# westlake-repl/IDvs.MoRec

Measured on AMD Instinct MI355X. Metric: user-sequences/sec end-to-end train step, SASRec+BERT-base, higher is better.
Workload: dtype fp16

## Files before the change

### idvs/morec_amd/_lib.py

```python
from __future__ import annotations

import ctypes as C
import os

import torch

_HERE = os.path.dirname(os.path.abspath(__file__))
LIB_PATH = os.environ.get("MOREC_HIP_LIB") or os.path.join(_HERE, "libmorec_hip.so")

F32, BF16, F16 = 0, 1, 2
ACT_NONE, ACT_GELU, ACT_RELU = 0, 1, 2
DACT_MUL = 3


class MorecError(RuntimeError):
    pass


class GemmDesc(C.Structure):
    _fields_ = [("M", C.c_int), ("N", C.c_int), ("K", C.c_int), ("lda", C.c_int), ("ldb", C.c_int), ("ldc", C.c_int),
                ("in_dtype", C.c_int), ("out_dtype", C.c_int), ("act", C.c_int), ("dact", C.c_int),
                ("accumulate", C.c_int), ("split_k", C.c_int), ("alpha", C.c_float), ("aux_deriv", C.c_int)]


# ... 17 lines not shown
    _fields_ = [("B", C.c_int), ("S", C.c_int), ("D", C.c_int), ("Nc", C.c_int), ("col_offset", C.c_int),
                ("dtype", C.c_int), ("dE_fp32", C.c_int), ("ws_from_fwd", C.c_int)]


class StepParams(C.Structure):
    _fields_ = [("step", C.c_int32), ("found_inf", C.c_int32), ("growth_tracker", C.c_int32), ("skipped", C.c_int32),
                ("loss_scale", C.c_float), ("inv_scale", C.c_float), ("bc1", C.c_float), ("bc2", C.c_float), ("apply", C.c_int32),
                ("pad0", C.c_int32), ("drop_seed", C.c_uint64), ("drop_seed_mixed", C.c_uint64), ("reserved", C.c_int32 * 2)]


class SwinAttnDesc(C.Structure):
    _fields_ = [("n_img", C.c_int), ("H", C.c_int), ("W", C.c_int), ("window", C.c_int), ("shift", C.c_int),
                ("heads", C.c_int), ("dh", C.c_int), ("scale", C.c_float), ("dtype", C.c_int)]


_P = C.c_void_p
_SIGS = {
    "morec_strerror": (C.c_char_p, [C.c_int]),
    "morec_version": (C.c_int, []),
    "morec_tuning_set": (C.c_int, [C.c_char_p, C.c_int]),
    "morec_det_scratch_reserve": (C.c_int, [C.c_size_t, C.c_void_p]),
    "morec_stream_wait_stream": (C.c_int, [_P, _P]),
    "morec_fold_defer_begin": (C.c_int, [_P]),
    "morec_fold_defer_active": (C.c_int, []),
    "morec_fold_flush": (C.c_int, [_P]),
    "morec_fold_defer_end": (C.c_int, []),
    "morec_fold_stats": (C.c_int, [_P]),
    "morec_gemm_nt": (C.c_int, [C.POINTER(GemmDesc), _P, _P, _P, _P, _P, _P, _P]),
    "morec_gemm_nt_colsum": (C.c_int, [C.POINTER(GemmDesc), _P, _P, _P, _P, _P, _P, _P, _P, _P]),
    "morec_gemm_colsum_workspace_bytes": (C.c_size_t, [C.c_int, C.c_int]),
    "morec_gemm_plan": (C.c_int, [C.POINTER(GemmDesc), C.c_int, C.c_int, C.c_int, C.c_int, C.c_int, C.POINTER(GemmPlanInfo)]),
    "morec_gemm_tn": (C.c_int, [_P, _P, _P, C.c_int, C.c_int, C.c_int, C.c_int, C.c_int, C.c_int, C.c_int, C.c_int, C.c_int, _P, _P]),
    "morec_gemm_tn_workspace_bytes": (C.c_size_t, [C.c_int, C.c_int, C.c_int]),
    "morec_mlp_dact_recompute_supported": (C.c_int, [C.c_int, C.c_int, C.c_int, C.c_int]),
    "morec_mlp_dact_recompute_workspace_bytes": (C.c_size_t, [C.c_int]),
    "morec_mlp_dact_recompute": (C.c_int, [_P, _P, _P, _P, _P, _P, _P, _P, C.c_int, C.c_int, C.c_int, C.c_int, _P]),
    "morec_transpose": (C.c_int, [_P, _P, C.c_int, C.c_int, C.c_int, C.c_int, C.c_int, C.c_int, _P]),
    "morec_transpose_batch": (C.c_int, [_P, C.c_int, C.c_int, C.c_int, _P]),
    "morec_cast": (C.c_int, [_P, _P, C.c_size_t, C.c_int, C.c_int, _P]),
    "morec_split_bf16x3": (C.c_int, [_P, _P, C.c_int, C.c_int, C.c_int, C.c_int, C.c_int, _P]),
    "morec_act_bwd": (C.c_int, [_P, _P, _P, C.c_size_t, C.c_int, C.c_int, _P]),
    "morec_scaled_sum": (C.c_int, [_P, _P, _P, _P, C.c_size_t, C.c_float, C.c_int, _P]),
    "morec_colsum": (C.c_int, [_P, _P, C.c_int, C.c_int, C.c_int, C.c_int, _P]),
    "morec_layernorm_fwd": (C.c_int, [_P, _P, _P, _P, C.c_int, _P, _P, C.c_float, _P, _P, _P, _P, C.c_int, C.c_int,
                                      C.c_int, C.c_float, C.c_uint64, C.c_float, C.c_uint64, _P, C.c_int, _P]),
    "morec_layernorm_bwd": (C.c_int, [_P, _P, _P, _P, _P, _P, _P, _P, _P, _P, _P, C.c_int, C.c_int, C.c_int, C.c_float,
                                      C.c_uint64, C.c_float, C.c_uint64, _P, _P, C.c_int, _P]),
    "morec_layernorm_fwd_res32": (C.c_int, [_P, _P, _P, _P, C.c_int, _P, _P, C.c_float, _P, _P, _P, _P, _P, C.c_int, C.c_int,
                                            C.c_int, C.c_float, C.c_uint64, C.c_float, C.c_uint64, _P]),
    "morec_layernorm_fwd_res32_pre": (C.c_int, [_P, _P, _P, _P, _P, _P, _P, _P, _P, C.c_float, _P, _P, _P, _P, C.c_int, C.c_int, C.c_int,
                                                C.c_float, C.c_uint64, _P]),
    "morec_layernorm_bwd_res32": (C.c_int, [_P, _P, _P, _P, _P, _P, _P, _P, _P, _P, _P, C.c_int, C.c_int, C.c_int, C.c_float,
                                            C.c_uint64, C.c_float, C.c_uint64, _P]),
    "morec_pos_grad": (C.c_int, [_P, _P, C.c_int, C.c_int, C.c_int, C.c_int, _P]),
    "morec_attn_fwd": (C.c_int, [C.POINTER(AttnDesc), _P, _P, _P, _P]),
    "morec_attn_bwd": (C.c_int, [C.POINTER(AttnDesc), _P, _P, _P, _P, _P]),
    "morec_attn_bwd_dbias": (C.c_int, [C.POINTER(AttnDesc), _P, _P, _P, _P, C.c_int, _P, _P, C.c_size_t, _P]),
    "morec_bert_embed_fwd": (C.c_int, [_P, _P, _P, _P, _P, _P, C.c_float, _P, _P, _P, _P, C.c_int, C.c_int, C.c_int,
                                       C.c_int, C.c_float, C.c_uint64, _P]),
    "morec_bert_embed_bwd": (C.c_int, [_P, _P, _P, _P, _P, C.c_int, C.c_int, C.c_int, C.c_int, C.c_int, _P, _P]),
    "morec_gather_rows": (C.c_int, [_P, _P, _P, C.c_int, C.c_int, C.c_int, _P]),
    "morec_scatter_add_rows": (C.c_int, [_P, _P, _P, C.c_int, C.c_int, C.c_int, C.c_int, _P]),
    "morec_indexed_rows_copy": (C.c_int, [_P, _P, _P, _P, C.c_int, C.c_int, C.c_int, _P]),
    "morec_strided_rows_copy": (C.c_int, [_P, _P, C.c_int, C.c_int, C.c_int, C.c_int, C.c_int, _P]),
    "morec_inbatch_ce_workspace_bytes": (C.c_size_t, [C.POINTER(CeDesc)]),
    "morec_inbatch_ce_fwd": (C.c_int, [C.POINTER(CeDesc), _P, _P, _P, _P, _P, _P, _P, _P, _P, _P, _P, _P]),
# ... 69 lines not shown
```

### idvs/morec_amd/csrc/gemm_tn.hip

```cpp
#include "gemm_core.hpp"
#include "gemm_args.hpp"

int gemm_tn8p_try_launch(const bf16* DY, const bf16* X, float* out, size_t slab_stride, int M, int N, int K, int ldy, int ldx, int ldo,
                         int mchunk, int zs, int dtype, hipStream_t s);

namespace {
constexpr int TT = 64;
constexpr int TC = 256;
constexpr int ROWB = TC * 2;
constexpr int OPB = TT * ROWB;
constexpr int STAGE = 2 * OPB;
constexpr int LDS_TN = 2 * STAGE;
constexpr int NWAVE = 16, NTHREADS = 1024;
constexpr int WN = 4, WK = 4;
constexpr int NI = 4, KI = 4;
constexpr int DPW = (TT * ROWB / 1024) / NWAVE;
typedef __attribute__((ext_vector_type(4))) short s16x4_t;
typedef __attribute__((address_space(3))) s16x4_t* lds_s16x4_ptr;

struct TnArgs {
    const bf16* DY;
    const bf16* X;
    float* C;
    int M, N, K, ldy, ldx, ldc, mchunk, tiles_n, tiles_k, atomic;
    float* slabs;
};

__device__ __forceinline__ bf16x8_t tr_frag(const char* tile, int ks, int blk) {
    const int lane = threadIdx.x & 63, c = lane & 15, g = lane >> 4;
    const int row = ks * 32 + 4 * g + (c >> 2);
    const char* p0 = tile + row * ROWB + ((blk ^ (row & 7)) * 32) + 8 * (c & 3);
    const s16x4_t lo = __builtin_amdgcn_ds_read_tr16_b64_v4i16((lds_s16x4_ptr)(p0));
    const s16x4_t hi = __builtin_amdgcn_ds_read_tr16_b64_v4i16((lds_s16x4_ptr)(p0 + 16 * ROWB));
    typedef __attribute__((ext_vector_type(8))) short s16x8_t;
    const s16x8_t v = {lo[0], lo[1], lo[2], lo[3], hi[0], hi[1], hi[2], hi[3]};
    return __builtin_bit_cast(bf16x8_t, v);
}
// ... 110 lines not shown
template <typename TO>
__global__ __launch_bounds__(256) void reduce_slabs_kernel(const float* __restrict__ slabs, TO* __restrict__ C, int N, int K,
                                                           int ldc, int nslab, int accumulate) {
    const size_t total4 = (size_t)N * K / 4;
    for (size_t i = blockIdx.x * (size_t)blockDim.x + threadIdx.x; i < total4; i += (size_t)gridDim.x * blockDim.x) {
        const size_t e = i * 4;
        const int n = (int)(e / K), k = (int)(e % K);
        float4 s = reinterpret_cast<const float4*>(slabs)[i];
        int t = 1;
        for (; t + 8 <= nslab; t += 8) {
            float4 v[8];
#pragma unroll
            for (int u = 0; u < 8; ++u) v[u] = reinterpret_cast<const float4*>(slabs + (size_t)(t + u) * N * K)[i];
#pragma unroll
            for (int u = 0; u < 8; ++u) { s.x += v[u].x; s.y += v[u].y; s.z += v[u].z; s.w += v[u].w; }
        }
        for (; t < nslab; ++t) {
            const float4 v = reinterpret_cast<const float4*>(slabs + (size_t)t * N * K)[i];
            s.x += v.x; s.y += v.y; s.z += v.z; s.w += v.w;
        }
        if constexpr (sizeof(TO) == 4) {
            float4* dst = reinterpret_cast<float4*>(C + (size_t)n * ldc + k);
            if (accumulate) {
                const float4 c = *dst;
                s.x += c.x; s.y += c.y; s.z += c.z; s.w += c.w;
            }
            *dst = s;
        } else {
            const float o[4] = {s.x, s.y, s.z, s.w};
            io<TO>::store4(C + (size_t)n * ldc + k, o);
        }
    }
}
}

extern "C" size_t morec_gemm_tn_workspace_bytes(int N, int K, int split_m) {
    return split_m > 1 ? (size_t)split_m * N * K * sizeof(float) : 0;
}

int gemm_tn_launch(const void* DY, const void* X, void* C, int c_dtype, int M, int N, int K, int ldy, int ldx, int ldc, int dtype, int split_m,
                   int accumulate, float* workspace, void* stream) {
    if (!DY || !X || !C || M <= 0 || N <= 0 || K <= 0) return MOREC_E_ARG;
    if (!is_h16(dtype)) return MOREC_E_UNSUPPORTED;
    if (c_dtype != MOREC_F32 && c_dtype != dtype) return MOREC_E_DTYPE;
    if (N % 8 || K % 8 || ldy % 8 || ldx % 8 || ldc % 4 || !aligned16(DY) || !aligned16(X) || !aligned16(C)) return MOREC_E_ALIGN;
    if (split_m > 1 && !accumulate && !workspace) return MOREC_E_ARG;
    TnArgs a;
    a.DY = reinterpret_cast<const bf16*>(DY); a.X = reinterpret_cast<const bf16*>(X); a.C = reinterpret_cast<float*>(C);
    a.M = M; a.N = N; a.K = K; a.ldy = ldy; a.ldx = ldx; a.ldc = ldc; a.atomic = accumulate ? 1 : 0;
    const int split = split_m < 1 ? 1 : split_m;
    int mchunk = (M + split - 1) / split;
    mchunk = ((mchunk + TT - 1) / TT) * TT;
    a.mchunk = mchunk;
    const int zs = (M + mchunk - 1) / mchunk;
    a.tiles_n = (N + TC - 1) / TC; a.tiles_k = (K + TC - 1) / TC;
    a.slabs = (zs > 1 && workspace) ? workspace : nullptr;
    if (a.slabs && (K % 4 || !aligned16(workspace))) return MOREC_E_ALIGN;
    if (c_dtype != MOREC_F32 && (!a.slabs || accumulate)) return MOREC_E_UNSUPPORTED;
    if (zs > 1 && !a.slabs && !accumulate) return MOREC_E_ARG;
    int r8 = MOREC_E_UNSUPPORTED;
    if (a.slabs)
        r8 = gemm_tn8p_try_launch(a.DY, a.X, a.slabs, (size_t)N * K, M, N, K, ldy, ldx, K, mchunk, zs, dtype, reinterpret_cast<hipStream_t>(stream));
    else if (zs == 1 && !accumulate)
        r8 = gemm_tn8p_try_launch(a.DY, a.X, a.C, 0, M, N, K, ldy, ldx, ldc, mchunk, 1, dtype, reinterpret_cast<hipStream_t>(stream));
    if (r8 != MOREC_E_UNSUPPORTED && r8 != MOREC_OK) return r8;
    if (r8 == MOREC_E_UNSUPPORTED) {
        by_h16(dtype, [&](auto* t) {
            using T = MOREC_TAG_T(t);
            static const hipError_t attr_rc = hipFuncSetAttribute(reinterpret_cast<const void*>(&gemm_tn_kernel<T>), hipFuncAttributeMaxDynamicSharedMemorySize, LDS_TN);
            (void)attr_rc;
            hipLaunchKernelGGL(gemm_tn_kernel<T>, dim3(a.tiles_n * a.tiles_k, 1, zs), dim3(NTHREADS), LDS_TN, reinterpret_cast<hipStream_t>(stream), a);
        });
        MOREC_CHECK_LAUNCH();
    }
    if (a.slabs) {
        const size_t total4 = (size_t)N * K / 4;
        const unsigned blocks = (unsigned)((total4 + 255) / 256 > 2048 ? 2048 : (total4 + 255) / 256);
        if (c_dtype == MOREC_F32)
            hipLaunchKernelGGL(reduce_slabs_kernel<float>, dim3(blocks), dim3(256), 0, reinterpret_cast<hipStream_t>(stream), a.slabs, a.C, N,
                               K, ldc, zs, accumulate ? 1 : 0);
        else if (c_dtype == MOREC_BF16)
            hipLaunchKernelGGL(reduce_slabs_kernel<bf16>, dim3(blocks), dim3(256), 0, reinterpret_cast<hipStream_t>(stream), a.slabs,
                               reinterpret_cast<bf16*>(C), N, K, ldc, zs, 0);
        else
            hipLaunchKernelGGL(reduce_slabs_kernel<f16>, dim3(blocks), dim3(256), 0, reinterpret_cast<hipStream_t>(stream), a.slabs,
                               reinterpret_cast<f16*>(C), N, K, ldc, zs, 0);
        MOREC_CHECK_LAUNCH();
// ... 9 lines not shown
```

### idvs/morec_amd/csrc/gemm_tn8p.hip

```cpp
#include "gemm_core.hpp"
#include "gemm_args.hpp"


namespace {
typedef __attribute__((ext_vector_type(16))) float f32x16_t;
typedef __attribute__((ext_vector_type(4))) unsigned int u32x4_t;
typedef __attribute__((ext_vector_type(4))) short s16x4_t;
typedef __attribute__((ext_vector_type(8))) short s16x8_t;
typedef __attribute__((address_space(3))) s16x4_t* lds_s16x4_ptr;

constexpr int TT = 64;
constexpr int ROWB = 256;
constexpr int HALF_BYTES = TT * ROWB;
constexpr int OP_BYTES = 2 * HALF_BYTES;
constexpr int BUF_BYTES = 2 * OP_BYTES;
constexpr int LDS_MAIN = 2 * BUF_BYTES;
constexpr int SLICE = 4096;
constexpr int LDS_TOTAL = LDS_MAIN + 8 * SLICE;
constexpr int THREADS = 512;

struct TnArgs8 {
    const bf16* DY;
    const bf16* X;
    float* out;
// ... 9 lines not shown
__device__ __forceinline__ void bar() {
    pin();
    __builtin_amdgcn_s_barrier();
    pin();
}
template <int REM, int W1, int W0>
__device__ __forceinline__ void vm_wait_tail() {
    vm_wait<(REM >= 2 ? 8 : (REM == 1 ? W1 : W0))>();
}

struct Ctx {
    __amdgpu_buffer_rsrc_t ry, rx;
    uint32_t y1[2], y2[2], x1[2], x2[2];
    int tok[2];
    int dpiece;
    int ay[2], ax;
    uint32_t vmask;
};

__device__ __forceinline__ void dma2(__amdgpu_buffer_rsrc_t rs, const uint32_t (&o)[2], const int (&tok)[2], int left, int soff, char* dst) {
    const uint32_t o0 = tok[0] < left ? o[0] : 0x80000000u;
    const uint32_t o1 = tok[1] < left ? o[1] : 0x80000000u;
    __builtin_amdgcn_raw_ptr_buffer_load_lds(rs, (lptr_t)dst, 16, o0, soff, 0, 0);
    __builtin_amdgcn_raw_ptr_buffer_load_lds(rs, (lptr_t)(dst + 1024), 16, o1, soff, 0, 0);
}

__device__ __forceinline__ bf16x8_t tr_frag(const char* smem, int addr, int ks) {
    const s16x4_t lo = __builtin_amdgcn_ds_read_tr16_b64_v4i16((lds_s16x4_ptr)(smem + addr + (16 * ks) * ROWB));
    const s16x4_t hi = __builtin_amdgcn_ds_read_tr16_b64_v4i16((lds_s16x4_ptr)(smem + addr + (16 * ks + 4) * ROWB));
    const s16x8_t v = {lo[0], lo[1], lo[2], lo[3], hi[0], hi[1], hi[2], hi[3]};
    return __builtin_bit_cast(bf16x8_t, v);
}

template <typename T16, int N0, int KQ, bool SKIP>
__device__ __forceinline__ void mfma_quadrant(f32x16_t (&acc)[4][2], const bf16x8_t (&fy)[2][4], const bf16x8_t (&fx)[4], uint32_t vm) {
    if constexpr (SKIP) {
        if (!(vm & (16u << KQ))) return;
        const bool a = (vm >> N0) & 1u, b = (vm >> (N0 + 1)) & 1u;
        if (!(a && b)) {
            if (!(a || b)) return;
            __builtin_amdgcn_s_setprio(1);
            if (a) {
#pragma unroll
                for (int ks = 0; ks < 4; ++ks) acc[N0][KQ] = h16<T16>::mma32(fx[ks], fy[0][ks], acc[N0][KQ]);
            } else {
#pragma unroll
                for (int ks = 0; ks < 4; ++ks) acc[N0 + 1][KQ] = h16<T16>::mma32(fx[ks], fy[1][ks], acc[N0 + 1][KQ]);
            }
            __builtin_amdgcn_s_setprio(0);
            return;
        }
    }
    __builtin_amdgcn_s_setprio(1);
#pragma unroll
    for (int ks = 0; ks < 4; ++ks)
#pragma unroll
        for (int ni = 0; ni < 2; ++ni)
            acc[N0 + ni][KQ] = h16<T16>::mma32(fx[ks], fy[ni][ks], acc[N0 + ni][KQ]);
    __builtin_amdgcn_s_setprio(0);
}

template <typename T16, int REM, bool SKIP>
__device__ __forceinline__ void stage(char* smem, const Ctx& c, int cb, int soy, int sox, int dy_step, int dx_step, int left,
                                      f32x16_t (&acc)[4][2]) {
    char* cur = smem + cb;
    char* oth = smem + (cb ^ BUF_BYTES);
    bf16x8_t fy[2][4], fx0[4], fx1[4];
    const int ay0 = cb + c.ay[0], ay1 = cb + c.ay[1], ax = cb + OP_BYTES + c.ax;
#pragma unroll
    for (int ks = 0; ks < 4; ++ks) fx0[ks] = tr_frag(smem, ax, ks);
#pragma unroll
    for (int ks = 0; ks < 4; ++ks) {
        fy[0][ks] = tr_frag(smem, ay0, ks);
        fy[1][ks] = tr_frag(smem, ay1, ks);
    }
    if constexpr (REM >= 1) dma2(c.rx, c.x2, c.tok, left - TT, sox + dx_step, oth + OP_BYTES + HALF_BYTES + c.dpiece);
    pin();
    vm_wait_tail<REM, 8, 2>();
    bar();
    mfma_quadrant<T16, 0, 0, SKIP>(acc, fy, fx0, c.vmask);
    bar();
#pragma unroll
    for (int ks = 0; ks < 4; ++ks) fx1[ks] = tr_frag(smem, ax + HALF_BYTES, ks);
    if constexpr (REM >= 1) dma2(c.ry, c.y2, c.tok, left - TT, soy + dy_step, oth + HALF_BYTES + c.dpiece);
    pin();
    vm_wait_tail<REM, 8, 0>();
    bar();
    mfma_quadrant<T16, 0, 1, SKIP>(acc, fy, fx1, c.vmask);
    bar();
#pragma unroll
    for (int ks = 0; ks < 4; ++ks) {
        fy[0][ks] = tr_frag(smem, ay0 + HALF_BYTES, ks);
        fy[1][ks] = tr_frag(smem, ay1 + HALF_BYTES, ks);
    }
    if constexpr (REM >= 2) dma2(c.ry, c.y1, c.tok, left - 2 * TT, soy + 2 * dy_step, cur + c.dpiece);
    pin();
    vm_wait_tail<REM, 6, 0>();
    bar();
    mfma_quadrant<T16, 2, 1, SKIP>(acc, fy, fx1, c.vmask);
    bar();
    if constexpr (REM >= 2) dma2(c.rx, c.x1, c.tok, left - 2 * TT, sox + 2 * dx_step, cur + OP_BYTES + c.dpiece);
    pin();
    vm_wait_tail<REM, 4, 0>();
    bar();
    mfma_quadrant<T16, 2, 0, SKIP>(acc, fy, fx0, c.vmask);
    bar();
}

template <typename T16, bool SKIP>
__device__ __forceinline__ void tn_body(const TnArgs8& p, char* smem, const bf16* __restrict__ DYt, const bf16* __restrict__ Xt, int n0, int k0,
                                        int mbeg, int mend, float* __restrict__ dst) {
    const int lane = threadIdx.x & 63;
    const int wave = __builtin_amdgcn_readfirstlane(threadIdx.x >> 6);
    const int wr = wave >> 2, wc = wave & 3;
    const int nt = (mend - mbeg + TT - 1) / TT;
    Ctx c;
    {
#pragma unroll
        for (int j = 0; j < 2; ++j) {
            const int t = 8 * wave + 4 * j + (lane >> 4);
            const int lc = (lane & 15) ^ (4 * (t & 3));
            const int ycol = (lc < 8 ? lc * 8 : 128 + (lc - 8) * 8);
            const int xcol = (lc >> 2) * 64 + (lc & 3) * 8;
            c.tok[j] = t;
            c.y1[j] = (uint32_t)(t * p.ldy + min(n0 + ycol, p.N - 8) - n0) * 2u;
            c.y2[j] = (uint32_t)(t * p.ldy + min(n0 + ycol + 64, p.N - 8) - n0) * 2u;
            c.x1[j] = (uint32_t)(t * p.ldx + min(k0 + xcol, p.K - 8) - k0) * 2u;
            c.x2[j] = (uint32_t)(t * p.ldx + min(k0 + xcol + 32, p.K - 8) - k0) * 2u;
        }
        const long ybytes = (long)(p.M - mbeg) * p.ldy * 2, xbytes = (long)(p.M - mbeg) * p.ldx * 2;
        c.ry = __builtin_amdgcn_make_buffer_rsrc((void*)DYt, 0, (int)min(ybytes, 0x7fffffffL), 0x00020000);
        c.rx = __builtin_amdgcn_make_buffer_rsrc((void*)Xt, 0, (int)min(xbytes, 0x7fffffffL), 0x00020000);
        c.dpiece = 8 * wave * ROWB;
        const int rr = (lane & 15) >> 2, cgrp = (lane >> 4) & 1, h = lane >> 5;
        const int rowoff = (8 * h + rr) * ROWB + 8 * (lane & 3);
#pragma unroll
        for (int cg = 0; cg < 2; ++cg) c.ay[cg] = rowoff + (((wr * 4 + cg * 2 + cgrp) ^ (2 * rr)) << 5);
        c.ax = rowoff + (((wc * 2 + cgrp) ^ (2 * rr)) << 5);
        uint32_t vm = 0;
#pragma unroll
        for (int i = 0; i < 4; ++i) vm |= (n0 + wr * 128 + i * 32 < p.N) ? (1u << i) : 0u;
#pragma unroll
        for (int j = 0; j < 2; ++j) vm |= (k0 + wc * 64 + j * 32 < p.K) ? (16u << j) : 0u;
        c.vmask = __builtin_amdgcn_readfirstlane(vm);
    }
    const int dy_step = TT * p.ldy * 2, dx_step = TT * p.ldx * 2;
    const int left0 = mend - mbeg;
    dma2(c.ry, c.y1, c.tok, left0, 0, smem + c.dpiece);
    dma2(c.rx, c.x1, c.tok, left0, 0, smem + OP_BYTES + c.dpiece);
    dma2(c.rx, c.x2, c.tok, left0, 0, smem + OP_BYTES + HALF_BYTES + c.dpiece);
    dma2(c.ry, c.y2, c.tok, left0, 0, smem + HALF_BYTES + c.dpiece);
    dma2(c.ry, c.y1, c.tok, left0 - TT, dy_step, smem + BUF_BYTES + c.dpiece);
    dma2(c.rx, c.x1, c.tok, left0 - TT, dx_step, smem + BUF_BYTES + OP_BYTES + c.dpiece);
    pin();

    f32x16_t acc[4][2];
#pragma unroll
    for (int i = 0; i < 4; ++i)
#pragma unroll
        for (int j = 0; j < 2; ++j)
#pragma unroll
            for (int v = 0; v < 16; ++v) acc[i][j][v] = 0.f;
    vm_wait<8>();
    bar();
    if (wr == 1) bar();
    int cb = 0, t = 0;
    for (; t < nt - 2; ++t) {
        stage<T16, 2, SKIP>(smem, c, cb, t * dy_step, t * dx_step, dy_step, dx_step, left0 - t * TT, acc);
        cb ^= BUF_BYTES;
    }
    stage<T16, 1, SKIP>(smem, c, cb, t * dy_step, t * dx_step, dy_step, dx_step, left0 - t * TT, acc);
    stage<T16, 0, SKIP>(smem, c, cb ^ BUF_BYTES, (t + 1) * dy_step, (t + 1) * dx_step, dy_step, dx_step, left0 - (t + 1) * TT, acc);
    if (wr == 0) bar();

    const int r5 = lane & 31, hh = lane >> 5;
    char* ws = smem + LDS_MAIN + wave * SLICE;
    const int rs_row = lane >> 3, rs_slot = lane & 7;
    const int rs_off = rs_row * 128 + ((rs_slot ^ (rs_row & 7)) << 4);
    const int nrows = min(256, p.N - n0);
    const long obytes = (long)nrows * p.ldo * 4;
    const __amdgpu_buffer_rsrc_t ro = __builtin_amdgcn_make_buffer_rsrc((void*)(dst + (size_t)n0 * p.ldo), 0, (int)min(obytes, 0x7fffffffL), 0x00020000);
    auto wfence = [&]() {
        __builtin_amdgcn_fence(__ATOMIC_RELEASE, "wavefront");
        __builtin_amdgcn_wave_barrier();
        __builtin_amdgcn_fence(__ATOMIC_ACQUIRE, "wavefront");
    };
#pragma unroll
    for (int Ni = 0; Ni < 4; ++Ni) {
#pragma unroll
        for (int Ki = 0; Ki < 2; ++Ki) {
            pin();
#pragma unroll
            for (int g = 0; g < 4; ++g) {
                const int slot = 2 * g + hh;
                *reinterpret_cast<float4*>(ws + r5 * 128 + ((slot ^ (r5 & 7)) << 4)) =
                    make_float4(acc[Ni][Ki][4 * g], acc[Ni][Ki][4 * g + 1], acc[Ni][Ki][4 * g + 2], acc[Ni][Ki][4 * g + 3]);
            }
            wfence();
            u32x4_t q[4];
#pragma unroll
            for (int i = 0; i < 4; ++i) q[i] = *reinterpret_cast<const u32x4_t*>(ws + rs_off + i * 1024);
            const int kcol = k0 + wc * 64 + Ki * 32 + rs_slot * 4;
            const uint32_t lo = kcol < p.K ? (uint32_t)((rs_row * p.ldo + kcol) * 4) : 0x80000000u;
#pragma unroll
            for (int i = 0; i < 4; ++i)
                __builtin_amdgcn_raw_buffer_store_b128(q[i], ro, lo + (uint32_t)((wr * 128 + Ni * 32 + 8 * i) * p.ldo * 4), 0, 0);
            wfence();
        }
    }
}

template <typename T16, bool SKIP>
__global__ __launch_bounds__(THREADS) void gemm_tn8p_kernel(TnArgs8 p) {
    extern __shared__ __attribute__((aligned(16))) char smem[];
    const int tiles = p.tiles_n * p.tiles_k;
    const int item = xcd_remap(blockIdx.x, tiles * p.zs);
    const int z = item / tiles, wg = item - z * tiles;
    const int n0 = (wg / p.tiles_k) * 256, k0 = (wg % p.tiles_k) * 256;
    const int mbeg = z * p.mchunk, mend = min(p.M, mbeg + p.mchunk);
    tn_body<T16, SKIP>(p, smem, p.DY + (size_t)mbeg * p.ldy + n0, p.X + (size_t)mbeg * p.ldx + k0, n0, k0, mbeg, mend,
            p.out + (size_t)z * p.slab_stride);
}
}

int gemm_tn8p_try_launch(const bf16* DY, const bf16* X, float* out, size_t slab_stride, int M, int N, int K, int ldy, int ldx, int ldo,
                         int mchunk, int zs, int dtype, hipStream_t s) {
    const int mode = tuning().gemm8p;
    if (mode == 1) return MOREC_E_UNSUPPORTED;
    if (N % 8 || K % 8 || ldo % 4) return MOREC_E_UNSUPPORTED;
    if (mchunk % TT || mchunk < 2 * TT) return MOREC_E_UNSUPPORTED;
    if (M - (zs - 1) * (long)mchunk < 2 * TT && zs > 1) return MOREC_E_UNSUPPORTED;
    if (zs == 1 && M < 2 * TT) return MOREC_E_UNSUPPORTED;
    const int tiles_n = (N + 255) / 256, tiles_k = (K + 255) / 256;
    if (mode != 2) {
        if (mchunk < 8 * TT) return MOREC_E_UNSUPPORTED;
    }
    if ((long)M * ldy * 2 >= 0x7fffffffL || (long)M * ldx * 2 >= 0x7fffffffL) return MOREC_E_UNSUPPORTED;
    TnArgs8 a;
    a.DY = DY; a.X = X; a.out = out; a.M = M; a.N = N; a.K = K; a.ldy = ldy; a.ldx = ldx; a.ldo = ldo; a.mchunk = mchunk;
    a.tiles_n = tiles_n; a.tiles_k = tiles_k; a.zs = zs; a.slab_stride = slab_stride;
    if (!by_h16(dtype, [&](auto* t) {
            using T = MOREC_TAG_T(t);
            static const hipError_t attr_rc = hipFuncSetAttribute(reinterpret_cast<const void*>(&gemm_tn8p_kernel<T, false>), hipFuncAttributeMaxDynamicSharedMemorySize, LDS_TOTAL);
            static const hipError_t attr_rc2 = hipFuncSetAttribute(reinterpret_cast<const void*>(&gemm_tn8p_kernel<T, true>), hipFuncAttributeMaxDynamicSharedMemorySize, LDS_TOTAL);
            (void)attr_rc; (void)attr_rc2;
            if (tuning().tn8p_skip && ((N % 256 != 0 && N % 256 <= 224) || (K % 256 != 0 && K % 256 <= 224)))
                hipLaunchKernelGGL((gemm_tn8p_kernel<T, true>), dim3(tiles_n * tiles_k * zs), dim3(THREADS), LDS_TOTAL, s, a);
            else
                hipLaunchKernelGGL((gemm_tn8p_kernel<T, false>), dim3(tiles_n * tiles_k * zs), dim3(THREADS), LDS_TOTAL, s, a);
        }))
        return MOREC_E_UNSUPPORTED;
    MOREC_CHECK_LAUNCH();
    return MOREC_OK;
}
```

### idvs/morec_amd/csrc/tuning.hip

```cpp
#include <stdlib.h>
#include <string.h>
#include "common.hpp"

namespace {
enum Handling {
    RAW,
    FLAG,
    TMR,
    RESERVE,
    TAIL_BIAS,
    MFMA,
    AT_LEAST_1,
    NOT_CHAR_0,
    IS_CHAR_1,
    EPI,
};
struct Row {
    const char* key;
    const char* env;
    int Tuning::*field;
    int def;
    Handling how;
};
const Row ROWS[] = {
    {"gemm8p", "MOREC_GEMM8P", &Tuning::gemm8p, 0, RAW},
    {"gemm2w", "MOREC_GEMM2W", &Tuning::gemm2w, 0, RAW},
    {"gemm_small", "MOREC_GEMM_SMALL", &Tuning::gemm_small, 0, RAW},
    {"gemm_skinny", "MOREC_GEMM_SKINNY", &Tuning::gemm_skinny, 0, RAW},
    {"ce8p", "MOREC_CE8P", &Tuning::ce8p, 0, RAW},
    {"gemm8p_tmr", "MOREC_GEMM8P_TMR", &Tuning::gemm8p_tmr, 1, TMR},
    {"gemm8p_ngroup", "MOREC_GEMM8P_NGROUP", &Tuning::gemm8p_ngroup, -1, RAW},
    {"gemm8p_reserve_cus", "MOREC_GEMM8P_RESERVE_CUS", &Tuning::gemm8p_reserve_cus, 0, RESERVE},
    {"gemm8p_tail_split", "MOREC_GEMM8P_TAIL_SPLIT", &Tuning::gemm8p_tail_split, 0, FLAG},
    {"gemm8p_tail_bias", nullptr, &Tuning::gemm8p_tail_bias, 2, TAIL_BIAS},
    {"gemm8p_mfma", "MOREC_GEMM8P_MFMA", &Tuning::gemm8p_mfma, 0, MFMA},
    {"gemm8p_debug", "MOREC_GEMM8P_DEBUG", &Tuning::gemm8p_debug, 0, RAW},
    {"gemm8p_stamps_lo", nullptr, &Tuning::gemm8p_stamps_lo, 0, RAW},
    {"gemm8p_stamps_hi", nullptr, &Tuning::gemm8p_stamps_hi, 0, RAW},
    {"deterministic", "MOREC_DETERMINISTIC", &Tuning::deterministic, 0, FLAG},
    {"fold_defer", "MOREC_FOLD_DEFER", &Tuning::fold_defer, 1, FLAG},
    {nullptr, "MOREC_GEMM_TILE", &Tuning::gemm_tile, 0, RAW},
    {nullptr, "MOREC_GEMM_EPI", &Tuning::gemm_epi, 2, EPI},
    {nullptr, "MOREC_GEMM2W_STAGGER", &Tuning::gemm2w_stagger, 0, RAW},
    {nullptr, "MOREC_TN8P_SKIP", &Tuning::tn8p_skip, 1, FLAG},
    {nullptr, "MOREC_ATTN_MFMA64", &Tuning::attn_mfma64, 1, NOT_CHAR_0},
    {nullptr, "MOREC_ATTN_F32_MFMA", &Tuning::attn_f32_mfma, 1, NOT_CHAR_0},
    {nullptr, "MOREC_SWIN_WPW_MIN", &Tuning::swin_wpw_min, 8, AT_LEAST_1},
    {nullptr, "MOREC_SWIN_BWD_WIDE", &Tuning::swin_bwd_wide, 1, RAW},
    {nullptr, "MOREC_QUIET", &Tuning::quiet, 0, IS_CHAR_1},
};

int handled(Handling how, int v) {
    switch (how) {
        case FLAG: return v != 0;
        case TMR: return (v == 0 || v == 1 || v == 224 || v == 192) ? v : 1;
        case RESERVE: return v < 0 ? 0 : v > 128 ? 128 : v;
        case TAIL_BIAS: return v < 0 ? 0 : v > 16 ? 16 : v;
        case MFMA: return (v == 16 || v == 32) ? v : 0;
        case AT_LEAST_1: return v < 1 ? 1 : v;
        default: return v;
    }
}

Tuning& table() {
    static Tuning t = [] {
        Tuning x{};
        for (const Row& r : ROWS) {
            const char* e = r.env ? getenv(r.env) : nullptr;
// ... 44 lines not shown
```

### idvs/morec_amd/csrc/tuning.hpp

```cpp
#pragma once

struct Tuning {
    int gemm8p, gemm2w, gemm_small, gemm_skinny, ce8p;
    int gemm8p_tmr;
    int gemm8p_ngroup;
    int gemm8p_reserve_cus;
    int gemm8p_tail_split, gemm8p_tail_bias;
    int gemm8p_mfma;
    int gemm8p_debug;
    int gemm8p_stamps_lo, gemm8p_stamps_hi;
    int deterministic;
    int fold_defer;
    int gemm_tile;
    int gemm_epi;
    int gemm2w_stagger;
    int tn8p_skip;
    int attn_mfma64;
    int attn_f32_mfma;
    int swin_wpw_min;
    int swin_bwd_wide;
    int quiet;

    unsigned long long gemm8p_stamps() const {
        return ((unsigned long long)(unsigned)gemm8p_stamps_hi << 32) | (unsigned)gemm8p_stamps_lo;
    }
};

const Tuning& tuning();

int device_cu_count();
int gemm8p_cu_count();
```

### include/morec_hip.h

```cpp
#ifndef MOREC_HIP_H
#define MOREC_HIP_H

#include <stddef.h>
#include <stdint.h>

#ifdef __cplusplus
extern "C" {
#endif

#define MOREC_F32 0
#define MOREC_BF16 1
#define MOREC_F16 2

#define MOREC_OK 0
#define MOREC_E_ARG (-1)
#define MOREC_E_ALIGN (-2)
#define MOREC_E_UNSUPPORTED (-3)
#define MOREC_E_DTYPE (-4)
#define MOREC_E_COMM (-5)

#define MOREC_ACT_NONE 0
#define MOREC_ACT_GELU 1
#define MOREC_ACT_RELU 2
#define MOREC_DACT_MUL 3
// ... 24 lines not shown
int morec_gemm_nt(const morec_gemm_desc* d, const void* A, const void* B, void* C, const float* bias,
                  void* aux_out, const void* dact_in, void* stream);

size_t morec_gemm_colsum_workspace_bytes(int M, int N);
int morec_gemm_nt_colsum(const morec_gemm_desc* d, const void* A, const void* B, void* C, const float* bias,
                         void* aux_out, const void* dact_in, float* colsum_out, float* workspace, void* stream);

#define MOREC_GEMM_UNSUPPORTED 0
#define MOREC_GEMM_SKINNY 1
#define MOREC_GEMM_SKINNY_WIDE 2
#define MOREC_GEMM_TWO_W 3
#define MOREC_GEMM_EIGHT_P 4
#define MOREC_GEMM_SMALL 5
#define MOREC_GEMM_GENERIC 6
typedef struct {
    int family;
    int mode;
    int tile_rows, tile_cols;
    int ngroup;
    int colsum_fused;
    const char* family_name;
} morec_gemm_plan_info;
int morec_gemm_plan(const morec_gemm_desc* d, int has_bias, int has_aux, int has_dact_in, int has_colsum, int n_cu,
                    morec_gemm_plan_info* out);

int morec_mlp_dact_recompute_supported(int M, int N, int K, int dtype);
size_t morec_mlp_dact_recompute_workspace_bytes(int N);
int morec_mlp_dact_recompute(const void* dY, const void* W2t, const void* X, const void* W1, const float* b1, void* dU,
                             float* colsum_out, float* workspace, int M, int N, int K, int dtype, void* stream);

int morec_gemm_tn(const void* DY, const void* X, float* C, int M, int N, int K, int ldy, int ldx, int ldc, int dtype,
                  int split_m, int accumulate, float* workspace, void* stream);
size_t morec_gemm_tn_workspace_bytes(int N, int K, int split_m);

int morec_transpose(const void* in, void* out, int R, int C, int ld_in, int ld_out, int in_dtype, int out_dtype,
                    void* stream);

typedef struct {
    const void* src;
    void* dst;
    int rows, cols;
    int ld_src, ld_dst;
    int tile0;
    int reserved;
} morec_transpose_item;
int morec_transpose_batch(const morec_transpose_item* items, int n_items, int n_tiles, int dtype, void* stream);
int morec_cast(const void* in, void* out, size_t n, int in_dtype, int out_dtype, void* stream);
int morec_split_bf16x3(const float* in, void* out, int R, int C, int ld_in, int ld_out, int lo_slot, void* stream);
int morec_act_bwd(const void* dy, const void* pre, void* out, size_t n, int act, int dtype, void* stream);
int morec_scaled_sum(const void* x0, const void* x1, const void* x2, void* out, size_t n, float scale, int dtype, void* stream);
int morec_colsum(const void* in, float* out, int M, int N, int ld, int dtype, void* stream);

int morec_layernorm_fwd(const void* x, const float* bias, const void* res, const float* pos, int pos_period,
                        const float* gamma, const float* beta, float eps, void* z_out, void* y, float* mean,
                        float* rstd, int M, int N, int dtype, float p_in, uint64_t seed_in, float p_out,
                        uint64_t seed_out, const float* rowscale, int rows_per_scale, void* stream);
int morec_layernorm_bwd(const void* dy_a, const void* dy_b, const void* z, const float* mean, const float* rstd,
                        const float* gamma, void* dz, void* dzd, float* dgamma, float* dbeta, float* dbias, int M, int N,
                        int dtype, float p_in, uint64_t seed_in, float p_out, uint64_t seed_out, const void* dres,
                        const float* rowscale, int rows_per_scale, void* stream);

int morec_layernorm_fwd_res32(const void* x16, const float* bias, const float* res32, const float* pos, int pos_period, const float* gamma,
                              const float* beta, float eps, float* z32, float* y32, void* y16, float* mean, float* rstd, int M, int N,
                              int dtype16, float p_in, uint64_t seed_in, float p_out, uint64_t seed_out, void* stream);
int morec_layernorm_fwd_res32_pre(const void* x16, const float* bias, const float* res_z32, const float* res_mean, const float* res_rstd,
                                  const float* res_gamma, const float* res_beta, const float* gamma, const float* beta, float eps, float* z32,
// ... 147 lines not shown
```

Baseline: 3720.

## Add 16x16 MFMA variant for TN weight-gradient GEMM kernel

Adds a 16x16x32 MFMA path to the 8-phase TN (weight-gradient) GEMM kernel. It brings new LDS transpose-read fragment addressing, a different swizzle, a split accumulator layout and its own epilogue store. An auto heuristic picks 16x16 for fp16, and for bf16 when the tile count is small. The skip-masked variant stays on 32x32. A plan query API and a tuning override are also exposed. The aim is better MFMA throughput or latency hiding for these shapes, at the cost of more LDS reads per MFMA and more kernel variants.

```diff
diff --git a/idvs/morec_amd/_lib.py b/idvs/morec_amd/_lib.py
--- a/idvs/morec_amd/_lib.py
+++ b/idvs/morec_amd/_lib.py
@@ -73,6 +73,7 @@
     "morec_gemm_plan": (C.c_int, [C.POINTER(GemmDesc), C.c_int, C.c_int, C.c_int, C.c_int, C.c_int, C.POINTER(GemmPlanInfo)]),
     "morec_gemm_tn": (C.c_int, [_P, _P, _P, C.c_int, C.c_int, C.c_int, C.c_int, C.c_int, C.c_int, C.c_int, C.c_int, C.c_int, _P, _P]),
     "morec_gemm_tn_workspace_bytes": (C.c_size_t, [C.c_int, C.c_int, C.c_int]),
+    "morec_gemm_tn_plan": (C.c_int, [C.c_int, C.c_int, C.c_int, C.c_int, C.c_int, C.POINTER(C.c_int), C.POINTER(C.c_int)]),
     "morec_mlp_dact_recompute_supported": (C.c_int, [C.c_int, C.c_int, C.c_int, C.c_int]),
     "morec_mlp_dact_recompute_workspace_bytes": (C.c_size_t, [C.c_int]),
     "morec_mlp_dact_recompute": (C.c_int, [_P, _P, _P, _P, _P, _P, _P, _P, C.c_int, C.c_int, C.c_int, C.c_int, _P]),
diff --git a/idvs/morec_amd/csrc/gemm_tn.hip b/idvs/morec_amd/csrc/gemm_tn.hip
--- a/idvs/morec_amd/csrc/gemm_tn.hip
+++ b/idvs/morec_amd/csrc/gemm_tn.hip
@@ -3,6 +3,7 @@
 
 int gemm_tn8p_try_launch(const bf16* DY, const bf16* X, float* out, size_t slab_stride, int M, int N, int K, int ldy, int ldx, int ldo,
                          int mchunk, int zs, int dtype, hipStream_t s);
+int gemm_tn8p_plan(int M, int N, int K, int ldy, int ldx, int ldo, int mchunk, int zs, int dtype, int* skip, int* mfma);
 
 namespace {
 constexpr int TT = 64;
@@ -179,6 +180,28 @@
         }
     }
 }
+inline void tn_chunks(int M, int split_m, int* mchunk, int* zs) {
+    const int split = split_m < 1 ? 1 : split_m;
+    int mc = (M + split - 1) / split;
+    mc = ((mc + TT - 1) / TT) * TT;
+    *mchunk = mc;
+    *zs = (M + mc - 1) / mc;
+}
+}
+
+extern "C" int morec_gemm_tn_plan(int M, int N, int K, int split_m, int dtype, int* family, int* mfma) {
+    if (M <= 0 || N <= 0 || K <= 0 || !family || !mfma) return MOREC_E_ARG;
+    *family = 0;
+    *mfma = 16;
+    if (!is_h16(dtype)) return MOREC_E_UNSUPPORTED;
+    if (N % 8 || K % 8) return MOREC_E_ALIGN;
+    int mchunk, zs, skip = 0, mf = 16;
+    tn_chunks(M, split_m, &mchunk, &zs);
+    if (gemm_tn8p_plan(M, N, K, N, K, K, mchunk, zs, dtype, &skip, &mf) == MOREC_OK) {
+        *family = skip ? 2 : 1;
+        *mfma = mf;
+    }
+    return MOREC_OK;
 }
 
 extern "C" size_t morec_gemm_tn_workspace_bytes(int N, int K, int split_m) {
@@ -195,11 +218,9 @@
     TnArgs a;
     a.DY = reinterpret_cast<const bf16*>(DY); a.X = reinterpret_cast<const bf16*>(X); a.C = reinterpret_cast<float*>(C);
     a.M = M; a.N = N; a.K = K; a.ldy = ldy; a.ldx = ldx; a.ldc = ldc; a.atomic = accumulate ? 1 : 0;
-    const int split = split_m < 1 ? 1 : split_m;
-    int mchunk = (M + split - 1) / split;
-    mchunk = ((mchunk + TT - 1) / TT) * TT;
+    int mchunk, zs;
+    tn_chunks(M, split_m, &mchunk, &zs);
     a.mchunk = mchunk;
-    const int zs = (M + mchunk - 1) / mchunk;
     a.tiles_n = (N + TC - 1) / TC; a.tiles_k = (K + TC - 1) / TC;
     a.slabs = (zs > 1 && workspace) ? workspace : nullptr;
     if (a.slabs && (K % 4 || !aligned16(workspace))) return MOREC_E_ALIGN;
diff --git a/idvs/morec_amd/csrc/gemm_tn8p.hip b/idvs/morec_amd/csrc/gemm_tn8p.hip
--- a/idvs/morec_amd/csrc/gemm_tn8p.hip
+++ b/idvs/morec_amd/csrc/gemm_tn8p.hip
@@ -65,15 +65,47 @@
     return __builtin_bit_cast(bf16x8_t, v);
 }
 
-template <typename T16, int N0, int KQ, bool SKIP>
-__device__ __forceinline__ void mfma_quadrant(f32x16_t (&acc)[4][2], const bf16x8_t (&fy)[2][4], const bf16x8_t (&fx)[4], uint32_t vm) {
+__device__ __forceinline__ bf16x8_t tr_frag16(const char* smem, int addr, int ks) {
+    const s16x4_t lo = __builtin_amdgcn_ds_read_tr16_b64_v4i16((lds_s16x4_ptr)(smem + addr + (32 * ks) * ROWB));
+    const s16x4_t hi = __builtin_amdgcn_ds_read_tr16_b64_v4i16((lds_s16x4_ptr)(smem + addr + (32 * ks + 16) * ROWB));
+    const s16x8_t v = {lo[0], lo[1], lo[2], lo[3], hi[0], hi[1], hi[2], hi[3]};
+    return __builtin_bit_cast(bf16x8_t, v);
+}
+template <int MF>
+__device__ __forceinline__ bf16x8_t frag(const char* smem, int addr, int i) {
+    if constexpr (MF == 32) return tr_frag(smem, addr, i);
+    else return tr_frag16(smem, addr ^ ((i & 1) << 5), i >> 1);
+}
+
+struct Acc16 {
+    f32x4_t q[4];
+};
+template <int MF>
+using acc_t = std::conditional_t<MF == 16, Acc16, f32x16_t>;
+
+template <typename T16, int NI0, int NIN, int KQ>
+__device__ __forceinline__ void mfma16_run(Acc16 (&acc)[4][2], const bf16x8_t (&fy)[2][4], const bf16x8_t (&fx)[4]) {
+#pragma unroll
+    for (int ks = 0; ks < 2; ++ks)
+#pragma unroll
+        for (int ni = NI0; ni < NI0 + NIN; ++ni)
+#pragma unroll
+            for (int sb = 0; sb < 4; ++sb)
+                acc[ni][KQ].q[sb] = h16<T16>::mma16(fx[2 * ks + (sb & 1)], fy[ni & 1][2 * ks + (sb >> 1)], acc[ni][KQ].q[sb]);
+}
+
+template <typename T16, int N0, int KQ, bool SKIP, int MF>
+__device__ __forceinline__ void mfma_quadrant(acc_t<MF> (&acc)[4][2], const bf16x8_t (&fy)[2][4], const bf16x8_t (&fx)[4], uint32_t vm) {
     if constexpr (SKIP) {
         if (!(vm & (16u << KQ))) return;
         const bool a = (vm >> N0) & 1u, b = (vm >> (N0 + 1)) & 1u;
         if (!(a && b)) {
             if (!(a || b)) return;
             __builtin_amdgcn_s_setprio(1);
-            if (a) {
+            if constexpr (MF == 16) {
+                if (a) mfma16_run<T16, N0, 1, KQ>(acc, fy, fx);
+                else mfma16_run<T16, N0 + 1, 1, KQ>(acc, fy, fx);
+            } else if (a) {
 #pragma unroll
                 for (int ks = 0; ks < 4; ++ks) acc[N0][KQ] = h16<T16>::mma32(fx[ks], fy[0][ks], acc[N0][KQ]);
             } else {
@@ -85,6 +117,8 @@
         }
     }
     __builtin_amdgcn_s_setprio(1);
+    if constexpr (MF == 16) mfma16_run<T16, N0, 2, KQ>(acc, fy, fx);
+    else
 #pragma unroll
     for (int ks = 0; ks < 4; ++ks)
 #pragma unroll
@@ -93,54 +127,54 @@
     __builtin_amdgcn_s_setprio(0);
 }
 
-template <typename T16, int REM, bool SKIP>
+template <typename T16, int REM, bool SKIP, int MF>
 __device__ __forceinline__ void stage(char* smem, const Ctx& c, int cb, int soy, int sox, int dy_step, int dx_step, int left,
-                                      f32x16_t (&acc)[4][2]) {
+                                      acc_t<MF> (&acc)[4][2]) {
     char* cur = smem + cb;
     char* oth = smem + (cb ^ BUF_BYTES);
     bf16x8_t fy[2][4], fx0[4], fx1[4];
     const int ay0 = cb + c.ay[0], ay1 = cb + c.ay[1], ax = cb + OP_BYTES + c.ax;
 #pragma unroll
-    for (int ks = 0; ks < 4; ++ks) fx0[ks] = tr_frag(smem, ax, ks);
+    for (int ks = 0; ks < 4; ++ks) fx0[ks] = frag<MF>(smem, ax, ks);
 #pragma unroll
     for (int ks = 0; ks < 4; ++ks) {
-        fy[0][ks] = tr_frag(smem, ay0, ks);
-        fy[1][ks] = tr_frag(smem, ay1, ks);
+        fy[0][ks] = frag<MF>(smem, ay0, ks);
+        fy[1][ks] = frag<MF>(smem, ay1, ks);
     }
     if constexpr (REM >= 1) dma2(c.rx, c.x2, c.tok, left - TT, sox + dx_step, oth + OP_BYTES + HALF_BYTES + c.dpiece);
     pin();
     vm_wait_tail<REM, 8, 2>();
     bar();
-    mfma_quadrant<T16, 0, 0, SKIP>(acc, fy, fx0, c.vmask);
-    bar();
-#pragma unroll
-    for (int ks = 0; ks < 4; ++ks) fx1[ks] = tr_frag(smem, ax + HALF_BYTES, ks);
+    mfma_quadrant<T16, 0, 0, SKIP, MF>(acc, fy, fx0, c.vmask);
+    bar();
+#pragma unroll
+    for (int ks = 0; ks < 4; ++ks) fx1[ks] = frag<MF>(smem, ax + HALF_BYTES, ks);
     if constexpr (REM >= 1) dma2(c.ry, c.y2, c.tok, left - TT, soy + dy_step, oth + HALF_BYTES + c.dpiece);
     pin();
     vm_wait_tail<REM, 8, 0>();
     bar();
-    mfma_quadrant<T16, 0, 1, SKIP>(acc, fy, fx1, c.vmask);
+    mfma_quadrant<T16, 0, 1, SKIP, MF>(acc, fy, fx1, c.vmask);
     bar();
 #pragma unroll
     for (int ks = 0; ks < 4; ++ks) {
-        fy[0][ks] = tr_frag(smem, ay0 + HALF_BYTES, ks);
-        fy[1][ks] = tr_frag(smem, ay1 + HALF_BYTES, ks);
+        fy[0][ks] = frag<MF>(smem, ay0 + HALF_BYTES, ks);
+        fy[1][ks] = frag<MF>(smem, ay1 + HALF_BYTES, ks);
     }
     if constexpr (REM >= 2) dma2(c.ry, c.y1, c.tok, left - 2 * TT, soy + 2 * dy_step, cur + c.dpiece);
     pin();
     vm_wait_tail<REM, 6, 0>();
     bar();
-    mfma_quadrant<T16, 2, 1, SKIP>(acc, fy, fx1, c.vmask);
+    mfma_quadrant<T16, 2, 1, SKIP, MF>(acc, fy, fx1, c.vmask);
     bar();
     if constexpr (REM >= 2) dma2(c.rx, c.x1, c.tok, left - 2 * TT, sox + 2 * dx_step, cur + OP_BYTES + c.dpiece);
     pin();
     vm_wait_tail<REM, 4, 0>();
     bar();
-    mfma_quadrant<T16, 2, 0, SKIP>(acc, fy, fx0, c.vmask);
-    bar();
-}
-
-template <typename T16, bool SKIP>
+    mfma_quadrant<T16, 2, 0, SKIP, MF>(acc, fy, fx0, c.vmask);
+    bar();
+}
+
+template <typename T16, bool SKIP, int MF>
 __device__ __forceinline__ void tn_body(const TnArgs8& p, char* smem, const bf16* __restrict__ DYt, const bf16* __restrict__ Xt, int n0, int k0,
                                         int mbeg, int mend, float* __restrict__ dst) {
     const int lane = threadIdx.x & 63;
@@ -152,7 +186,7 @@
 #pragma unroll
         for (int j = 0; j < 2; ++j) {
             const int t = 8 * wave + 4 * j + (lane >> 4);
-            const int lc = (lane & 15) ^ (4 * (t & 3));
+            const int lc = (lane & 15) ^ (MF == 16 ? 2 * (t & 7) : 4 * (t & 3));
             const int ycol = (lc < 8 ? lc * 8 : 128 + (lc - 8) * 8);
             const int xcol = (lc >> 2) * 64 + (lc & 3) * 8;
             c.tok[j] = t;
@@ -165,11 +199,19 @@
         c.ry = __builtin_amdgcn_make_buffer_rsrc((void*)DYt, 0, (int)min(ybytes, 0x7fffffffL), 0x00020000);
         c.rx = __builtin_amdgcn_make_buffer_rsrc((void*)Xt, 0, (int)min(xbytes, 0x7fffffffL), 0x00020000);
         c.dpiece = 8 * wave * ROWB;
+        if constexpr (MF == 16) {
+            const int row = 4 * (lane >> 4) + ((lane & 15) >> 2);
+            const int rowoff = row * ROWB + 8 * (lane & 3);
+#pragma unroll
+            for (int cg = 0; cg < 2; ++cg) c.ay[cg] = rowoff + (((wr * 4 + cg * 2) ^ (row & 7)) << 5);
+            c.ax = rowoff + (((wc * 2) ^ (row & 7)) << 5);
+        } else {
         const int rr = (lane & 15) >> 2, cgrp = (lane >> 4) & 1, h = lane >> 5;
         const int rowoff = (8 * h + rr) * ROWB + 8 * (lane & 3);
 #pragma unroll
         for (int cg = 0; cg < 2; ++cg) c.ay[cg] = rowoff + (((wr * 4 + cg * 2 + cgrp) ^ (2 * rr)) << 5);
         c.ax = rowoff + (((wc * 2 + cgrp) ^ (2 * rr)) << 5);
+        }
         uint32_t vm = 0;
 #pragma unroll
         for (int i = 0; i < 4; ++i) vm |= (n0 + wr * 128 + i * 32 < p.N) ? (1u << i) : 0u;
@@ -187,23 +229,26 @@
     dma2(c.rx, c.x1, c.tok, left0 - TT, dx_step, smem + BUF_BYTES + OP_BYTES + c.dpiece);
     pin();
 
-    f32x16_t acc[4][2];
+    acc_t<MF> acc[4][2];
 #pragma unroll
     for (int i = 0; i < 4; ++i)
 #pragma unroll
         for (int j = 0; j < 2; ++j)
 #pragma unroll
-            for (int v = 0; v < 16; ++v) acc[i][j][v] = 0.f;
+            for (int v = 0; v < 16; ++v) {
+                if constexpr (MF == 16) acc[i][j].q[v >> 2][v & 3] = 0.f;
+                else acc[i][j][v] = 0.f;
+            }
     vm_wait<8>();
     bar();
     if (wr == 1) bar();
     int cb = 0, t = 0;
     for (; t < nt - 2; ++t) {
-        stage<T16, 2, SKIP>(smem, c, cb, t * dy_step, t * dx_step, dy_step, dx_step, left0 - t * TT, acc);
+        stage<T16, 2, SKIP, MF>(smem, c, cb, t * dy_step, t * dx_step, dy_step, dx_step, left0 - t * TT, acc);
         cb ^= BUF_BYTES;
     }
-    stage<T16, 1, SKIP>(smem, c, cb, t * dy_step, t * dx_step, dy_step, dx_step, left0 - t * TT, acc);
-    stage<T16, 0, SKIP>(smem, c, cb ^ BUF_BYTES, (t + 1) * dy_step, (t + 1) * dx_step, dy_step, dx_step, left0 - (t + 1) * TT, acc);
+    stage<T16, 1, SKIP, MF>(smem, c, cb, t * dy_step, t * dx_step, dy_step, dx_step, left0 - t * TT, acc);
+    stage<T16, 0, SKIP, MF>(smem, c, cb ^ BUF_BYTES, (t + 1) * dy_step, (t + 1) * dx_step, dy_step, dx_step, left0 - (t + 1) * TT, acc);
     if (wr == 0) bar();
 
     const int r5 = lane & 31, hh = lane >> 5;
@@ -223,12 +268,21 @@
 #pragma unroll
         for (int Ki = 0; Ki < 2; ++Ki) {
             pin();
+            if constexpr (MF == 16) {
+#pragma unroll
+                for (int sb = 0; sb < 4; ++sb) {
+                    const int row = 16 * (sb >> 1) + (lane & 15), slot = 4 * (sb & 1) + (lane >> 4);
+                    *reinterpret_cast<float4*>(ws + row * 128 + ((slot ^ (row & 7)) << 4)) =
+                        make_float4(acc[Ni][Ki].q[sb][0], acc[Ni][Ki].q[sb][1], acc[Ni][Ki].q[sb][2], acc[Ni][Ki].q[sb][3]);
+                }
+            } else {
 #pragma unroll
             for (int g = 0; g < 4; ++g) {
                 const int slot = 2 * g + hh;
                 *reinterpret_cast<float4*>(ws + r5 * 128 + ((slot ^ (r5 & 7)) << 4)) =
                     make_float4(acc[Ni][Ki][4 * g], acc[Ni][Ki][4 * g + 1], acc[Ni][Ki][4 * g + 2], acc[Ni][Ki][4 * g + 3]);
             }
+            }
             wfence();
             u32x4_t q[4];
 #pragma unroll
@@ -243,7 +297,7 @@
     }
 }
 
-template <typename T16, bool SKIP>
+template <typename T16, bool SKIP, int MF>
 __global__ __launch_bounds__(THREADS) void gemm_tn8p_kernel(TnArgs8 p) {
     extern __shared__ __attribute__((aligned(16))) char smem[];
     const int tiles = p.tiles_n * p.tiles_k;
@@ -251,36 +305,65 @@
     const int z = item / tiles, wg = item - z * tiles;
     const int n0 = (wg / p.tiles_k) * 256, k0 = (wg % p.tiles_k) * 256;
     const int mbeg = z * p.mchunk, mend = min(p.M, mbeg + p.mchunk);
-    tn_body<T16, SKIP>(p, smem, p.DY + (size_t)mbeg * p.ldy + n0, p.X + (size_t)mbeg * p.ldx + k0, n0, k0, mbeg, mend,
+    tn_body<T16, SKIP, MF>(p, smem, p.DY + (size_t)mbeg * p.ldy + n0, p.X + (size_t)mbeg * p.ldx + k0, n0, k0, mbeg, mend,
             p.out + (size_t)z * p.slab_stride);
 }
 }
 
-int gemm_tn8p_try_launch(const bf16* DY, const bf16* X, float* out, size_t slab_stride, int M, int N, int K, int ldy, int ldx, int ldo,
-                         int mchunk, int zs, int dtype, hipStream_t s) {
-    const int mode = tuning().gemm8p;
+static int tn8p_mfma_auto(int N, int K, int dtype, int skip) {
+    if (skip) return 32;
+    if (dtype == MOREC_F16) return 16;
+    return ((N + 255) / 256) * ((K + 255) / 256) <= 9 ? 16 : 32;
+}
+
+int gemm_tn8p_plan(int M, int N, int K, int ldy, int ldx, int ldo, int mchunk, int zs, int dtype, int* skip, int* mfma) {
+    const Tuning& t = tuning();
+    const int mode = t.gemm8p;
     if (mode == 1) return MOREC_E_UNSUPPORTED;
+    if (!is_h16(dtype)) return MOREC_E_UNSUPPORTED;
     if (N % 8 || K % 8 || ldo % 4) return MOREC_E_UNSUPPORTED;
     if (mchunk % TT || mchunk < 2 * TT) return MOREC_E_UNSUPPORTED;
     if (M - (zs - 1) * (long)mchunk < 2 * TT && zs > 1) return MOREC_E_UNSUPPORTED;
     if (zs == 1 && M < 2 * TT) return MOREC_E_UNSUPPORTED;
-    const int tiles_n = (N + 255) / 256, tiles_k = (K + 255) / 256;
     if (mode != 2) {
         if (mchunk < 8 * TT) return MOREC_E_UNSUPPORTED;
     }
     if ((long)M * ldy * 2 >= 0x7fffffffL || (long)M * ldx * 2 >= 0x7fffffffL) return MOREC_E_UNSUPPORTED;
+    *skip = t.tn8p_skip && ((N % 256 != 0 && N % 256 <= 224) || (K % 256 != 0 && K % 256 <= 224));
+    *mfma = t.gemm_tn8p_mfma ? t.gemm_tn8p_mfma : tn8p_mfma_auto(N, K, dtype, *skip);
+    return MOREC_OK;
+}
+
+int gemm_tn8p_try_launch(const bf16* DY, const bf16* X, float* out, size_t slab_stride, int M, int N, int K, int ldy, int ldx, int ldo,
+                         int mchunk, int zs, int dtype, hipStream_t s) {
+    int skip = 0, mfma = 32;
+    if (gemm_tn8p_plan(M, N, K, ldy, ldx, ldo, mchunk, zs, dtype, &skip, &mfma) != MOREC_OK) return MOREC_E_UNSUPPORTED;
+    const int tiles_n = (N + 255) / 256, tiles_k = (K + 255) / 256;
     TnArgs8 a;
     a.DY = DY; a.X = X; a.out = out; a.M = M; a.N = N; a.K = K; a.ldy = ldy; a.ldx = ldx; a.ldo = ldo; a.mchunk = mchunk;
     a.tiles_n = tiles_n; a.tiles_k = tiles_k; a.zs = zs; a.slab_stride = slab_stride;
+    auto launch = [&](auto kernel) {
+        hipLaunchKernelGGL(kernel, dim3(tiles_n * tiles_k * zs), dim3(THREADS), LDS_TOTAL, s, a);
+    };
     if (!by_h16(dtype, [&](auto* t) {
             using T = MOREC_TAG_T(t);
-            static const hipError_t attr_rc = hipFuncSetAttribute(reinterpret_cast<const void*>(&gemm_tn8p_kernel<T, false>), hipFuncAttributeMaxDynamicSharedMemorySize, LDS_TOTAL);
-            static const hipError_t attr_rc2 = hipFuncSetAttribute(reinterpret_cast<const void*>(&gemm_tn8p_kernel<T, true>), hipFuncAttributeMaxDynamicSharedMemorySize, LDS_TOTAL);
-            (void)attr_rc; (void)attr_rc2;
-            if (tuning().tn8p_skip && ((N % 256 != 0 && N % 256 <= 224) || (K % 256 != 0 && K % 256 <= 224)))
-                hipLaunchKernelGGL((gemm_tn8p_kernel<T, true>), dim3(tiles_n * tiles_k * zs), dim3(THREADS), LDS_TOTAL, s, a);
-            else
-                hipLaunchKernelGGL((gemm_tn8p_kernel<T, false>), dim3(tiles_n * tiles_k * zs), dim3(THREADS), LDS_TOTAL, s, a);
+            static const hipError_t attr_rc = [] {
+                hipError_t rc = hipSuccess;
+                for (const void* k : {reinterpret_cast<const void*>(&gemm_tn8p_kernel<T, false, 32>), reinterpret_cast<const void*>(&gemm_tn8p_kernel<T, true, 32>),
+                                      reinterpret_cast<const void*>(&gemm_tn8p_kernel<T, false, 16>), reinterpret_cast<const void*>(&gemm_tn8p_kernel<T, true, 16>)}) {
+                    const hipError_t r = hipFuncSetAttribute(k, hipFuncAttributeMaxDynamicSharedMemorySize, LDS_TOTAL);
+                    if (r != hipSuccess) rc = r;
+                }
+                return rc;
+            }();
+            (void)attr_rc;
+            if (mfma == 16) {
+                if (skip) launch(gemm_tn8p_kernel<T, true, 16>);
+                else launch(gemm_tn8p_kernel<T, false, 16>);
+            } else {
+                if (skip) launch(gemm_tn8p_kernel<T, true, 32>);
+                else launch(gemm_tn8p_kernel<T, false, 32>);
+            }
         }))
         return MOREC_E_UNSUPPORTED;
     MOREC_CHECK_LAUNCH();
diff --git a/idvs/morec_amd/csrc/tuning.hip b/idvs/morec_amd/csrc/tuning.hip
--- a/idvs/morec_amd/csrc/tuning.hip
+++ b/idvs/morec_amd/csrc/tuning.hip
@@ -34,6 +34,7 @@
     {"gemm8p_tail_split", "MOREC_GEMM8P_TAIL_SPLIT", &Tuning::gemm8p_tail_split, 0, FLAG},
     {"gemm8p_tail_bias", nullptr, &Tuning::gemm8p_tail_bias, 2, TAIL_BIAS},
     {"gemm8p_mfma", "MOREC_GEMM8P_MFMA", &Tuning::gemm8p_mfma, 0, MFMA},
+    {"gemm_tn8p_mfma", "MOREC_GEMM_TN8P_MFMA", &Tuning::gemm_tn8p_mfma, 0, MFMA},
     {"gemm8p_debug", "MOREC_GEMM8P_DEBUG", &Tuning::gemm8p_debug, 0, RAW},
     {"gemm8p_stamps_lo", nullptr, &Tuning::gemm8p_stamps_lo, 0, RAW},
     {"gemm8p_stamps_hi", nullptr, &Tuning::gemm8p_stamps_hi, 0, RAW},
diff --git a/idvs/morec_amd/csrc/tuning.hpp b/idvs/morec_amd/csrc/tuning.hpp
--- a/idvs/morec_amd/csrc/tuning.hpp
+++ b/idvs/morec_amd/csrc/tuning.hpp
@@ -7,6 +7,7 @@
     int gemm8p_reserve_cus;
     int gemm8p_tail_split, gemm8p_tail_bias;
     int gemm8p_mfma;
+    int gemm_tn8p_mfma;
     int gemm8p_debug;
     int gemm8p_stamps_lo, gemm8p_stamps_hi;
     int deterministic;
diff --git a/include/morec_hip.h b/include/morec_hip.h
--- a/include/morec_hip.h
+++ b/include/morec_hip.h
@@ -80,6 +80,7 @@
 int morec_gemm_tn(const void* DY, const void* X, float* C, int M, int N, int K, int ldy, int ldx, int ldc, int dtype,
                   int split_m, int accumulate, float* workspace, void* stream);
 size_t morec_gemm_tn_workspace_bytes(int N, int K, int split_m);
+int morec_gemm_tn_plan(int M, int N, int K, int split_m, int dtype, int* family, int* mfma);
 
 int morec_transpose(const void* in, void* out, int R, int C, int ld_in, int ld_out, int in_dtype, int out_dtype,
                     void* stream);
```

Measured after the change: 3725, median of 4. Within noise of the previous version (+0.2%).
